# ByteDance-Seed/Bagel

Hardware: NVIDIA H100
Metric: denoised images/sec @1024^2, 50 steps, BAGEL-7B-MoT (higher is better)
Workload: dtype bf16

## Files before the change

### bagel_b200/csrc/attn.cu

```cuda
#include <cuda.h>
#include <cuda_bf16.h>
#include <cuda_runtime.h>
#include <stdint.h>
#include <stdio.h>
#include <stdlib.h>

#include "common.cuh"
#include "host_util.h"
#include "attn_decode.h"

namespace bagel {

constexpr int kAttnThreads = 2 * 128 + 32;
constexpr int kAttnMmaWarps = 8;
constexpr int kBlockM = 128;
constexpr int kBlockN = 128;

struct AttnParams {
  __nv_bfloat16* out;
  long long ld_out;
  const int* cu_q;
  const int* cu_k;
  const int* seqused_k;
  int Hq, Hk;
  int causal;
  float scale_log2;
  int poly;
};

template <int D>
struct AttnCfg {
  static constexpr int kTileBytes = kBlockM * D * 2;
  static constexpr int kStages = (D == 128) ? 4 : 6;
  static constexpr int kSmemBytes = kTileBytes + kStages * kTileBytes + 1024 + 256;
};

__device__ __forceinline__ float ex2(float x) {
  float y;
  asm("ex2.approx.ftz.f32 %0, %1;" : "=f"(y) : "f"(x));
  return y;
}

__device__ __forceinline__ float2 ex2_poly2(float2 x) {
  const float2 magic = make_float2(12582912.0f, 12582912.0f);
  const float2 c1 = make_float2(0.69328292f, 0.69328292f), c2 = make_float2(0.24221068f, 0.24221068f),
               c3 = make_float2(0.05500873f, 0.05500873f);
  x.x = fmaxf(x.x, -126.0f);
  x.y = fmaxf(x.y, -126.0f);
  const float2 t = make_float2(x.x + magic.x, x.y + magic.y);
  const float2 n = make_float2(t.x - magic.x, t.y - magic.y);
  const float2 f = make_float2(x.x - n.x, x.y - n.y);
  float2 q = make_float2(fmaf(f.x, c3.x, c2.x), fmaf(f.y, c3.y, c2.y));
  q = make_float2(fmaf(q.x, f.x, c1.x), fmaf(q.y, f.y, c1.y));
  q = make_float2(fmaf(q.x, f.x, 1.0f), fmaf(q.y, f.y, 1.0f));
  float2 r;
  r.x = __int_as_float(__float_as_int(q.x) + (__float_as_int(t.x) << 23));
  r.y = __int_as_float(__float_as_int(q.y) + (__float_as_int(t.y) << 23));
  return r;
}

template <int D>
__global__ void __launch_bounds__(kAttnThreads, 1)
attn_varlen_kernel(const __grid_constant__ CUtensorMap tmQ, const __grid_constant__ CUtensorMap tmK,
                   const __grid_constant__ CUtensorMap tmV, const AttnParams p) {
  using Cfg = AttnCfg<D>;
  constexpr int kStages = Cfg::kStages;
  constexpr int kTileBytes = Cfg::kTileBytes;
  constexpr int kAtoms = D / 64;
  constexpr int kAtomBytes = kBlockM * 128;

  const int qt = p.causal ? (int)(gridDim.x - 1 - blockIdx.x) : (int)blockIdx.x;
  const int h = blockIdx.y, b = blockIdx.z;
  const int q_beg = p.cu_q[b];
  const int Lq = p.cu_q[b + 1] - q_beg;
  const int q0 = qt * kBlockM;
  if (q0 >= Lq) return;
  const int hk = h / (p.Hq / p.Hk);
  const int k_beg = p.cu_k[b];
  const int Lk = p.seqused_k ? p.seqused_k[b] : (p.cu_k[b + 1] - k_beg);
  const int shift = Lk - Lq;
  int kv_end = Lk;
  if (p.causal) kv_end = max(0, min(Lk, min(Lq, q0 + kBlockM) - 1 + shift + 1));
  const int nblk = (kv_end + kBlockN - 1) / kBlockN;

  extern __shared__ uint8_t smem_raw[];
  uint8_t* smem = reinterpret_cast<uint8_t*>((reinterpret_cast<uintptr_t>(smem_raw) + 1023) & ~uintptr_t(1023));
  uint8_t* smem_q = smem;
  uint8_t* smem_kv = smem + kTileBytes;
  uint64_t* bars = reinterpret_cast<uint64_t*>(smem_kv + kStages * kTileBytes);
  uint64_t* q_full = bars;
  uint64_t* kv_full = bars + 1;
  uint64_t* kv_empty = kv_full + kStages;

  const int wg = threadIdx.x >> 7;
  const int warp = threadIdx.x >> 5;
  const int lane = threadIdx.x & 31;

  if (threadIdx.x == 0) {
    tma_prefetch_desc(&tmQ);
    tma_prefetch_desc(&tmK);
    tma_prefetch_desc(&tmV);
    mbar_init(q_full, 1);
    for (int i = 0; i < kStages; ++i) {
      mbar_init(&kv_full[i], 1);
      mbar_init(&kv_empty[i], kAttnMmaWarps);
    }
    fence_mbar_init();
  }
  __syncthreads();

  if (wg == 2) {
    if (elect_one_lane() && nblk > 0) {
      mbar_expect_tx(q_full, kTileBytes);
      for (int a = 0; a < kAtoms; ++a)
        tma_load_2d(smem_q + a * kAtomBytes, &tmQ, q_full, h * D + a * 64, q_beg + q0, kEvictFirst);
      int stage = 0;
      uint32_t phase = 0;
      for (int j = 0; j < nblk; ++j) {
        for (int kv = 0; kv < 2; ++kv) {
          mbar_wait(&kv_empty[stage], phase ^ 1);
          mbar_expect_tx(&kv_full[stage], kTileBytes);
          const CUtensorMap* tm = kv == 0 ? &tmK : &tmV;
          for (int a = 0; a < kAtoms; ++a)
            tma_load_2d(smem_kv + stage * kTileBytes + a * kAtomBytes, tm, &kv_full[stage], hk * D + a * 64,
                        k_beg + j * kBlockN, kEvictLast);
          if (++stage == kStages) { stage = 0; phase ^= 1; }
        }
      }
    }
  } else {
    const int half = wg;
    const int cq = 2 * (lane & 3);
    const int row0 = half * 64 + (warp & 3) * 16 + (lane >> 2);
    const int qi[2] = {q0 + row0, q0 + row0 + 8};
    float o[D / 2];
#pragma unroll
    for (int i = 0; i < D / 2; ++i) o[i] = 0.f;
    float m[2] = {-INFINITY, -INFINITY}, l[2] = {0.f, 0.f};

    if (nblk > 0) {
      mbar_wait(q_full, 0);
      const uint32_t q_addr = smem_u32(smem_q) + half * 64 * 128;
      const int tile_q_lo = q0 + half * 64;
      int stage = 0;
      uint32_t phase = 0;
      for (int j = 0; j < nblk; ++j) {
        float s[kBlockN / 2];
        mbar_wait(&kv_full[stage], phase);
        {
          const uint32_t k_addr = smem_u32(smem_kv + stage * kTileBytes);
          wgmma_fence();
#pragma unroll
          for (int a = 0; a < kAtoms; ++a)
#pragma unroll
            for (int k = 0; k < 4; ++k)
              wgmma_ss<kBlockN>(s, gmma_desc_kmajor_sw128(q_addr + a * kAtomBytes) + 2 * k,
                                gmma_desc_kmajor_sw128(k_addr + a * kAtomBytes) + 2 * k, (a | k) != 0);
          wgmma_commit();
          wgmma_wait<0>();
          gmma_fence_operand(s);
        }
        __syncwarp();
        if (lane == 0) mbar_arrive(&kv_empty[stage]);
        if (++stage == kStages) { stage = 0; phase ^= 1; }

        const int kv0 = j * kBlockN;
        const bool need_mask = (kv0 + kBlockN > Lk) || (p.causal && (kv0 + kBlockN - 1 > tile_q_lo + shift));
        if (need_mask) {
#pragma unroll
          for (int r = 0; r < 2; ++r) {
            const int lim = p.causal ? min(Lk - 1, qi[r] + shift) : (Lk - 1);
#pragma unroll
            for (int c = 0; c < kBlockN / 8; ++c)
#pragma unroll
              for (int e = 0; e < 2; ++e)
                if (kv0 + 8 * c + cq + e > lim) s[4 * c + 2 * r + e] = -INFINITY;
          }
        }
        float neg_ms[2], alpha[2];
#pragma unroll
        for (int r = 0; r < 2; ++r) {
          float mx = -INFINITY;
#pragma unroll
          for (int c = 0; c < kBlockN / 8; ++c) mx = fmaxf(mx, fmaxf(s[4 * c + 2 * r], s[4 * c + 2 * r + 1]));
          mx = fmaxf(mx, __shfl_xor_sync(0xffffffffu, mx, 1));
          mx = fmaxf(mx, __shfl_xor_sync(0xffffffffu, mx, 2));
          const float m_new = fmaxf(m[r], mx);
          const float m_use = (m_new == -INFINITY) ? 0.f : m_new;
          alpha[r] = ex2((m[r] - m_use) * p.scale_log2);
          m[r] = m_new;
          neg_ms[r] = -m_use * p.scale_log2;
        }
        const bool poly = p.poly && !need_mask;
        float rs[2] = {0.f, 0.f};
        uint32_t pa[kBlockN / 16][4];
#pragma unroll
        for (int c = 0; c < kBlockN / 8; ++c) {
#pragma unroll
          for (int r = 0; r < 2; ++r) {
            const float2 x = make_float2(fmaf(s[4 * c + 2 * r], p.scale_log2, neg_ms[r]),
                                         fmaf(s[4 * c + 2 * r + 1], p.scale_log2, neg_ms[r]));
            const float2 e = (poly && (c & 3) == 3) ? ex2_poly2(x) : make_float2(ex2(x.x), ex2(x.y));
            rs[r] += e.x + e.y;
            pa[c >> 1][(c & 1) * 2 + r] = pack_bf16x2(e.x, e.y);
          }
        }
#pragma unroll
        for (int r = 0; r < 2; ++r) {
          l[r] = l[r] * alpha[r] + rs[r];
#pragma unroll
          for (int c = 0; c < D / 8; ++c) {
            o[4 * c + 2 * r] *= alpha[r];
            o[4 * c + 2 * r + 1] *= alpha[r];
          }
        }

        mbar_wait(&kv_full[stage], phase);
        {
          const uint32_t v_addr = smem_u32(smem_kv + stage * kTileBytes);
          wgmma_fence();
#pragma unroll
          for (int kk = 0; kk < kBlockN / 16; ++kk)
            wgmma_rs<D, 1>(o, pa[kk], gmma_desc_mnmajor_sw128(v_addr + kk * 2048, kAtomBytes), 1u);
          wgmma_commit();
          wgmma_wait<0>();
          gmma_fence_operand(o);
        }
        __syncwarp();
        if (lane == 0) mbar_arrive(&kv_empty[stage]);
        if (++stage == kStages) { stage = 0; phase ^= 1; }
      }
    }

#pragma unroll
    for (int r = 0; r < 2; ++r) {
      float lr = l[r];
      lr += __shfl_xor_sync(0xffffffffu, lr, 1);
      lr += __shfl_xor_sync(0xffffffffu, lr, 2);
      const float inv_l = (lr > 0.f && m[r] != -INFINITY) ? (1.f / lr) : 0.f;
      if (qi[r] >= Lq) continue;
      __nv_bfloat16* orow = p.out + (long long)(q_beg + qi[r]) * p.ld_out + h * D;
#pragma unroll
      for (int c = 0; c < D / 8; ++c)
        *reinterpret_cast<uint32_t*>(orow + 8 * c + cq) = pack_bf16x2(o[4 * c + 2 * r] * inv_l, o[4 * c + 2 * r + 1] * inv_l);
    }
  }
}

template <int D>
static int launch_attn(const CUtensorMap& tmQ, const CUtensorMap& tmK, const CUtensorMap& tmV, const AttnParams& p, int B,
                       int max_seqlen_q, cudaStream_t stream) {
  using Cfg = AttnCfg<D>;
  auto kern = attn_varlen_kernel<D>;
  static bool attr_done = false;
  if (!attr_done) {
    BAGEL_CUDA_CHECK(cudaFuncSetAttribute(kern, cudaFuncAttributeMaxDynamicSharedMemorySize, Cfg::kSmemBytes));
    attr_done = true;
  }
  const int qtiles = (max_seqlen_q + kBlockM - 1) / kBlockM;
  if (p.Hq > 65535 || B > 65535) return set_error(BAGEL_ERR_SHAPE, "bagel_attn_varlen_fwd: too many heads / samples");
  kern<<<dim3(qtiles, p.Hq, B), kAttnThreads, Cfg::kSmemBytes, stream>>>(tmQ, tmK, tmV, p);
  g_launches.fetch_add(1, std::memory_order_relaxed);
  BAGEL_CUDA_CHECK(cudaGetLastError());
  return 0;
}

}

using namespace bagel;

extern "C" int bagel_attn_varlen_fwd(const void* q, const void* k, const void* v, void* out, const int* cu_seqlens_q,
                                     const int* cu_seqlens_k, int total_q, int total_k, int batch, int num_heads_q,
                                     int num_heads_k, int head_dim, int max_seqlen_q, int max_seqlen_k, int causal,
                                     float softmax_scale, long long ld_q, long long ld_k, long long ld_v,
                                     long long ld_out, const int* seqused_k, void* stream) {
  if (head_dim != 64 && head_dim != 128)
    return set_error(BAGEL_ERR_SHAPE, "bagel_attn_varlen_fwd: head_dim must be 64 or 128 (got %d)", head_dim);
  if (num_heads_k <= 0 || num_heads_q % num_heads_k)
    return set_error(BAGEL_ERR_SHAPE, "bagel_attn_varlen_fwd: num_heads_q %% num_heads_k != 0");
  if (batch <= 0 || total_q < 0 || total_k < 0) return set_error(BAGEL_ERR_SHAPE, "bagel_attn_varlen_fwd: bad sizes");
  if ((ld_q % 8) || (ld_k % 8) || (ld_v % 8) || (ld_out % 8) || (((uintptr_t)q | (uintptr_t)k | (uintptr_t)v | (uintptr_t)out) & 15))
    return set_error(BAGEL_ERR_ALIGN, "bagel_attn_varlen_fwd: row strides %% 8 and 16-byte aligned pointers required");
  if (int rc = require_sm90()) return rc;
  if (total_q == 0 || max_seqlen_q <= 0) return 0;
  if (attn_decode_supported(max_seqlen_q, head_dim, num_heads_q, num_heads_k))
    return attn_decode(q, k, v, out, cu_seqlens_q, cu_seqlens_k, seqused_k, batch, num_heads_q, num_heads_k,
                       max_seqlen_k, softmax_scale, ld_q, ld_k, ld_v, ld_out, static_cast<cudaStream_t>(stream));

  CUtensorMap tmQ, tmK, tmV;
  if (int rc = make_tmap_2d_bf16(&tmQ, q, (uint64_t)num_heads_q * head_dim, (uint64_t)total_q, (uint64_t)ld_q, 64, kBlockM)) return rc;
  const uint64_t rows_k = total_k > 0 ? (uint64_t)total_k : 1;
  if (int rc = make_tmap_2d_bf16(&tmK, k, (uint64_t)num_heads_k * head_dim, rows_k, (uint64_t)ld_k, 64, kBlockN)) return rc;
  if (int rc = make_tmap_2d_bf16(&tmV, v, (uint64_t)num_heads_k * head_dim, rows_k, (uint64_t)ld_v, 64, kBlockN)) return rc;

  AttnParams p{};
  p.out = static_cast<__nv_bfloat16*>(out);
  p.ld_out = ld_out;
  p.cu_q = cu_seqlens_q;
  p.cu_k = cu_seqlens_k;
  p.seqused_k = seqused_k;
  p.Hq = num_heads_q;
  p.Hk = num_heads_k;
  p.causal = causal;
  p.scale_log2 = softmax_scale * 1.4426950408889634f;
  static const int poly_env = [] { const char* e = getenv("BAGEL_ATTN_POLY"); return e ? (atoi(e) != 0 ? 1 : 0) : -1; }();
  p.poly = poly_env >= 0 ? poly_env : ((causal || max_seqlen_k < 2048) ? 0 : 1);
  cudaStream_t s = static_cast<cudaStream_t>(stream);
  if (head_dim == 128) return launch_attn<128>(tmQ, tmK, tmV, p, batch, max_seqlen_q, s);
  return launch_attn<64>(tmQ, tmK, tmV, p, batch, max_seqlen_q, s);
}
```

### bagel_b200/csrc/common.cuh

```cuda
#pragma once
#include <cuda.h>
#include <cuda_bf16.h>
#include <cuda_runtime.h>
#include <stdint.h>
#include <stdio.h>

#include "wgmma.cuh"

namespace bagel {

__device__ __forceinline__ uint32_t smem_u32(const void* p) {
  return static_cast<uint32_t>(__cvta_generic_to_shared(p));
}

__device__ __forceinline__ bool elect_one() {
  uint32_t pred = 0;
  asm volatile(
      "{\n\t"
      ".reg .pred P;\n\t"
      "elect.sync _|P, 0xffffffff;\n\t"
      "selp.b32 %0, 1, 0, P;\n\t"
      "}\n"
      : "=r"(pred));
  return pred != 0;
}

__device__ __forceinline__ void mbar_init(uint64_t* bar, uint32_t count) {
  asm volatile("mbarrier.init.shared::cta.b64 [%0], %1;" ::"r"(smem_u32(bar)), "r"(count) : "memory");
}
__device__ __forceinline__ void fence_mbar_init() {
  asm volatile("fence.mbarrier_init.release.cluster;" ::: "memory");
}
__device__ __forceinline__ void mbar_expect_tx(uint64_t* bar, uint32_t bytes) {
  asm volatile("mbarrier.arrive.expect_tx.shared::cta.b64 _, [%0], %1;" ::"r"(smem_u32(bar)), "r"(bytes)
               : "memory");
}
__device__ __forceinline__ void mbar_arrive(uint64_t* bar) {
  asm volatile("mbarrier.arrive.shared::cta.b64 _, [%0];" ::"r"(smem_u32(bar)) : "memory");
}
__device__ __forceinline__ bool mbar_try_wait(uint64_t* bar, uint32_t parity) {
  uint32_t ok;
  asm volatile(
      "{\n\t"
      ".reg .pred P;\n\t"
      "mbarrier.try_wait.parity.shared::cta.b64 P, [%1], %2;\n\t"
      "selp.b32 %0, 1, 0, P;\n\t"
      "}\n"
      : "=r"(ok)
      : "r"(smem_u32(bar)), "r"(parity)
      : "memory");
  return ok != 0;
}
__device__ __forceinline__ void mbar_wait(uint64_t* bar, uint32_t parity) {
  if (mbar_try_wait(bar, parity)) return;
  const long long t0 = clock64();
  while (!mbar_try_wait(bar, parity)) {
    if (clock64() - t0 > 4000000000LL) {
#ifdef BAGEL_MBAR_TRACE
      printf("bagel_b200: mbarrier wait timed out (block %d thread %d bar %u parity %u)\n", blockIdx.x,
             threadIdx.x, smem_u32(bar), parity);
#endif
      __trap();
    }
  }
}

__device__ __forceinline__ uint32_t cluster_ctarank() {
  uint32_t r;
  asm volatile("mov.u32 %0, %%cluster_ctarank;" : "=r"(r));
  return r;
}
__device__ __forceinline__ void cluster_sync_all() {
  asm volatile("barrier.cluster.arrive.release.aligned;" ::: "memory");
  asm volatile("barrier.cluster.wait.acquire.aligned;" ::: "memory");
}
__device__ __forceinline__ uint32_t mapa_shared(uint32_t local_addr, uint32_t rank) {
  uint32_t remote;
  asm volatile("mapa.shared::cluster.u32 %0, %1, %2;" : "=r"(remote) : "r"(local_addr), "r"(rank));
  return remote;
}
__device__ __forceinline__ float ld_dsmem_f32(uint32_t local_addr, uint32_t rank) {
  float v;
  asm volatile("ld.shared::cluster.f32 %0, [%1];" : "=f"(v) : "r"(mapa_shared(local_addr, rank)) : "memory");
  return v;
}
__device__ __forceinline__ void mbar_arrive_cluster(uint64_t* bar, uint32_t rank) {
  asm volatile("mbarrier.arrive.shared::cluster.b64 _, [%0];" ::"r"(mapa_shared(smem_u32(bar), rank)) : "memory");
}

__device__ __forceinline__ bool elect_one_lane() {
  uint32_t pred;
  asm volatile(
      "{\n\t"
      ".reg .pred p;\n\t"
      "elect.sync _|p, 0xffffffff;\n\t"
      "selp.b32 %0, 1, 0, p;\n\t"
      "}\n"
      : "=r"(pred));
  return pred != 0;
}

__device__ __forceinline__ void pdl_launch_dependents() { asm volatile("griddepcontrol.launch_dependents;" ::: "memory"); }
__device__ __forceinline__ void pdl_wait() { asm volatile("griddepcontrol.wait;" ::: "memory"); }

__device__ __forceinline__ void fence_async_smem() {
  asm volatile("fence.proxy.async.shared::cta;" ::: "memory");
}

__device__ __forceinline__ void tma_prefetch_desc(const CUtensorMap* tm) {
  asm volatile("prefetch.tensormap [%0];" ::"l"(reinterpret_cast<uint64_t>(tm)) : "memory");
}
constexpr uint64_t kEvictNormal = 0x1000000000000000ull;
constexpr uint64_t kEvictFirst = 0x12F0000000000000ull;
constexpr uint64_t kEvictLast = 0x14F0000000000000ull;

__device__ __forceinline__ void tma_load_2d(void* smem_dst, const CUtensorMap* tm, uint64_t* bar, int c0, int c1,
                                            uint64_t hint) {
  asm volatile(
      "cp.async.bulk.tensor.2d.shared::cluster.global.mbarrier::complete_tx::bytes.L2::cache_hint"
      " [%0], [%1, {%3, %4}], [%2], %5;"
      ::"r"(smem_u32(smem_dst)),
      "l"(reinterpret_cast<uint64_t>(tm)), "r"(smem_u32(bar)), "r"(c0), "r"(c1), "l"(hint)
      : "memory");
}
__device__ __forceinline__ void tma_load_2d_multicast(void* smem_dst, const CUtensorMap* tm, uint64_t* bar, int c0, int c1,
                                                      uint16_t cta_mask, uint64_t hint) {
  asm volatile(
      "cp.async.bulk.tensor.2d.shared::cluster.global.mbarrier::complete_tx::bytes.multicast::cluster.L2::cache_hint"
      " [%0], [%1, {%3, %4}], [%2], %5, %6;"
      ::"r"(smem_u32(smem_dst)),
      "l"(reinterpret_cast<uint64_t>(tm)), "r"(smem_u32(bar)), "r"(c0), "r"(c1), "h"(cta_mask), "l"(hint)
      : "memory");
}
__device__ __forceinline__ void tma_load_4d(void* smem_dst, const CUtensorMap* tm, uint64_t* bar, int c0, int c1,
                                            int c2, int c3, uint64_t hint) {
  asm volatile(
      "cp.async.bulk.tensor.4d.shared::cluster.global.mbarrier::complete_tx::bytes.L2::cache_hint"
      " [%0], [%1, {%3, %4, %5, %6}], [%2], %7;"
      ::"r"(smem_u32(smem_dst)),
      "l"(reinterpret_cast<uint64_t>(tm)), "r"(smem_u32(bar)), "r"(c0), "r"(c1), "r"(c2), "r"(c3), "l"(hint)
      : "memory");
}
__device__ __forceinline__ void tma_store_2d(const CUtensorMap* tm, const void* smem_src, int c0, int c1) {
  asm volatile("cp.async.bulk.tensor.2d.global.shared::cta.bulk_group [%0, {%2, %3}], [%1];" ::"l"(
                   reinterpret_cast<uint64_t>(tm)),
               "r"(smem_u32(smem_src)), "r"(c0), "r"(c1)
               : "memory");
}
__device__ __forceinline__ void tma_store_commit() { asm volatile("cp.async.bulk.commit_group;" ::: "memory"); }
template <int N>
__device__ __forceinline__ void tma_store_wait_read() {
  asm volatile("cp.async.bulk.wait_group.read %0;" ::"n"(N) : "memory");
}
template <int N>
__device__ __forceinline__ void tma_store_wait() {
  asm volatile("cp.async.bulk.wait_group %0;" ::"n"(N) : "memory");
}

__device__ __forceinline__ uint64_t gmma_desc_kmajor_sw128(uint32_t smem_addr) {
  return (uint64_t)((smem_addr & 0x3FFFF) >> 4) | (1ull << 16) | ((uint64_t)(1024 >> 4) << 32) | (1ull << 62);
}
__device__ __forceinline__ uint64_t gmma_desc_mnmajor_sw128(uint32_t smem_addr, uint32_t lbo_bytes) {
  return (uint64_t)((smem_addr & 0x3FFFF) >> 4) | ((uint64_t)((lbo_bytes >> 4) & 0x3FFF) << 16) |
         ((uint64_t)(1024 >> 4) << 32) | (1ull << 62);
}

template <int N>
__device__ __forceinline__ void gmma_fence_operand(float (&d)[N]) {
#pragma unroll
  for (int i = 0; i < N; ++i) asm volatile("" : "+f"(d[i])::"memory");
}
__device__ __forceinline__ void wgmma_fence() { asm volatile("wgmma.fence.sync.aligned;" ::: "memory"); }
__device__ __forceinline__ void wgmma_commit() { asm volatile("wgmma.commit_group.sync.aligned;" ::: "memory"); }
template <int N>
__device__ __forceinline__ void wgmma_wait() {
  asm volatile("wgmma.wait_group.sync.aligned %0;" ::"n"(N) : "memory");
}

template <int N, int kTnspB = 0>
__device__ __forceinline__ void wgmma_ss(float (&d)[N / 2], uint64_t a_desc, uint64_t b_desc, uint32_t scale_d) {
  if constexpr (N == 16) wgmma_ss_n16<kTnspB>(d, a_desc, b_desc, scale_d);
  else if constexpr (N == 32) wgmma_ss_n32<kTnspB>(d, a_desc, b_desc, scale_d);
  else if constexpr (N == 64) wgmma_ss_n64<kTnspB>(d, a_desc, b_desc, scale_d);
  else if constexpr (N == 128) wgmma_ss_n128<kTnspB>(d, a_desc, b_desc, scale_d);
  else {
    static_assert(N == 256, "wgmma_ss: N in {16, 32, 64, 128, 256}");
    wgmma_ss_n256<kTnspB>(d, a_desc, b_desc, scale_d);
  }
}
template <int N, int kTnspB>
__device__ __forceinline__ void wgmma_rs(float (&d)[N / 2], const uint32_t (&a)[4], uint64_t b_desc, uint32_t scale_d) {
  if constexpr (N == 64) wgmma_rs_n64<kTnspB>(d, a, b_desc, scale_d);
  else {
    static_assert(N == 128, "wgmma_rs: N in {64, 128}");
    wgmma_rs_n128<kTnspB>(d, a, b_desc, scale_d);
  }
}

template <uint32_t kRegs>
__device__ __forceinline__ void setmaxnreg_dec() { asm volatile("setmaxnreg.dec.sync.aligned.u32 %0;" ::"n"(kRegs)); }
template <uint32_t kRegs>
__device__ __forceinline__ void setmaxnreg_inc() { asm volatile("setmaxnreg.inc.sync.aligned.u32 %0;" ::"n"(kRegs)); }

__device__ __forceinline__ float bf16_round(float x) { return __bfloat162float(__float2bfloat16_rn(x)); }
__device__ __forceinline__ uint32_t pack_bf16x2(float lo, float hi) {
  __nv_bfloat162 v = __floats2bfloat162_rn(lo, hi);
  return *reinterpret_cast<uint32_t*>(&v);
}
__device__ __forceinline__ float bf16_lo(uint32_t v) { return __uint_as_float(v << 16); }
__device__ __forceinline__ float bf16_hi(uint32_t v) { return __uint_as_float(v & 0xFFFF0000u); }

}
```

Before: 0.09359.

## Make varlen attention persistent with Q double-use barriers and ping-pong warpgroup scheduling

Converts the attention kernel into a persistent kernel launched with one CTA per SM that loops over flattened (qtile, head, batch) tiles. A q_empty barrier lets the producer reload Q for the next tile while K/V keep streaming. Named barriers alternate the two consumer warpgroups' QK^T wgmma issue so one group's softmax overlaps the other's tensor-core work. This removes per-CTA launch and prologue overhead, but adds barrier handshakes, a required even stage count, and extra paths for inactive half-tiles.

```diff
diff --git a/bagel_b200/csrc/attn.cu b/bagel_b200/csrc/attn.cu
--- a/bagel_b200/csrc/attn.cu
+++ b/bagel_b200/csrc/attn.cu
@@ -1,6 +1,7 @@
 #include <cuda.h>
 #include <cuda_bf16.h>
 #include <cuda_runtime.h>
+#include <limits.h>
 #include <stdint.h>
 #include <stdio.h>
 #include <stdlib.h>
@@ -23,6 +24,9 @@
   const int* cu_k;
   const int* seqused_k;
   int Hq, Hk;
+  int batch;
+  int qtiles;
+  int ntiles;
   int causal;
   float scale_log2;
   int poly;
@@ -59,6 +63,42 @@
   return r;
 }
 
+struct AttnTile {
+  int h, b, hk;
+  int q_beg, Lq, q0;
+  int k_beg, Lk;
+  int shift;
+  int nblk;
+};
+
+__device__ __forceinline__ bool attn_tile(const AttnParams& p, int t, AttnTile& g) {
+  int qt;
+  if (p.causal) {
+    const int hb = p.Hq * p.batch;
+    qt = p.qtiles - 1 - t / hb;
+    t %= hb;
+  } else {
+    qt = t % p.qtiles;
+    t /= p.qtiles;
+  }
+  g.h = t % p.Hq;
+  g.b = t / p.Hq;
+  g.q_beg = p.cu_q[g.b];
+  g.Lq = p.cu_q[g.b + 1] - g.q_beg;
+  g.q0 = qt * kBlockM;
+  if (g.q0 >= g.Lq) return false;
+  g.hk = g.h / (p.Hq / p.Hk);
+  g.k_beg = p.cu_k[g.b];
+  g.Lk = p.seqused_k ? p.seqused_k[g.b] : (p.cu_k[g.b + 1] - g.k_beg);
+  g.shift = g.Lk - g.Lq;
+  int kv_end = g.Lk;
+  if (p.causal) kv_end = max(0, min(g.Lk, min(g.Lq, g.q0 + kBlockM) - 1 + g.shift + 1));
+  g.nblk = (kv_end + kBlockN - 1) / kBlockN;
+  return true;
+}
+
+constexpr uint32_t kBarTurn = 1;
+
 template <int D>
 __global__ void __launch_bounds__(kAttnThreads, 1)
 attn_varlen_kernel(const __grid_constant__ CUtensorMap tmQ, const __grid_constant__ CUtensorMap tmK,
@@ -68,20 +108,7 @@
   constexpr int kTileBytes = Cfg::kTileBytes;
   constexpr int kAtoms = D / 64;
   constexpr int kAtomBytes = kBlockM * 128;
-
-  const int qt = p.causal ? (int)(gridDim.x - 1 - blockIdx.x) : (int)blockIdx.x;
-  const int h = blockIdx.y, b = blockIdx.z;
-  const int q_beg = p.cu_q[b];
-  const int Lq = p.cu_q[b + 1] - q_beg;
-  const int q0 = qt * kBlockM;
-  if (q0 >= Lq) return;
-  const int hk = h / (p.Hq / p.Hk);
-  const int k_beg = p.cu_k[b];
-  const int Lk = p.seqused_k ? p.seqused_k[b] : (p.cu_k[b + 1] - k_beg);
-  const int shift = Lk - Lq;
-  int kv_end = Lk;
-  if (p.causal) kv_end = max(0, min(Lk, min(Lq, q0 + kBlockM) - 1 + shift + 1));
-  const int nblk = (kv_end + kBlockN - 1) / kBlockN;
+  static_assert(kStages % 2 == 0, "K_j and V_j share a ring phase: K at an even stage, V at the next one");
 
   extern __shared__ uint8_t smem_raw[];
   uint8_t* smem = reinterpret_cast<uint8_t*>((reinterpret_cast<uintptr_t>(smem_raw) + 1023) & ~uintptr_t(1023));
@@ -89,7 +116,8 @@
   uint8_t* smem_kv = smem + kTileBytes;
   uint64_t* bars = reinterpret_cast<uint64_t*>(smem_kv + kStages * kTileBytes);
   uint64_t* q_full = bars;
-  uint64_t* kv_full = bars + 1;
+  uint64_t* q_empty = bars + 1;
+  uint64_t* kv_full = bars + 2;
   uint64_t* kv_empty = kv_full + kStages;
 
   const int wg = threadIdx.x >> 7;
@@ -101,6 +129,7 @@
     tma_prefetch_desc(&tmK);
     tma_prefetch_desc(&tmV);
     mbar_init(q_full, 1);
+    mbar_init(q_empty, kAttnMmaWarps);
     for (int i = 0; i < kStages; ++i) {
       mbar_init(&kv_full[i], 1);
       mbar_init(&kv_empty[i], kAttnMmaWarps);
@@ -110,145 +139,178 @@
   __syncthreads();
 
   if (wg == 2) {
-    if (elect_one_lane() && nblk > 0) {
-      mbar_expect_tx(q_full, kTileBytes);
-      for (int a = 0; a < kAtoms; ++a)
-        tma_load_2d(smem_q + a * kAtomBytes, &tmQ, q_full, h * D + a * 64, q_beg + q0, kEvictFirst);
+    if (elect_one_lane()) {
       int stage = 0;
-      uint32_t phase = 0;
-      for (int j = 0; j < nblk; ++j) {
-        for (int kv = 0; kv < 2; ++kv) {
-          mbar_wait(&kv_empty[stage], phase ^ 1);
-          mbar_expect_tx(&kv_full[stage], kTileBytes);
-          const CUtensorMap* tm = kv == 0 ? &tmK : &tmV;
-          for (int a = 0; a < kAtoms; ++a)
-            tma_load_2d(smem_kv + stage * kTileBytes + a * kAtomBytes, tm, &kv_full[stage], hk * D + a * 64,
-                        k_beg + j * kBlockN, kEvictLast);
-          if (++stage == kStages) { stage = 0; phase ^= 1; }
+      uint32_t phase = 0, q_phase = 0;
+      for (int t = blockIdx.x; t < p.ntiles; t += gridDim.x) {
+        AttnTile g;
+        if (!attn_tile(p, t, g) || g.nblk == 0) continue;
+        mbar_wait(q_empty, q_phase ^ 1);
+        q_phase ^= 1;
+        mbar_expect_tx(q_full, kTileBytes);
+        for (int a = 0; a < kAtoms; ++a)
+          tma_load_2d(smem_q + a * kAtomBytes, &tmQ, q_full, g.h * D + a * 64, g.q_beg + g.q0, kEvictFirst);
+        for (int j = 0; j < g.nblk; ++j) {
+          for (int kv = 0; kv < 2; ++kv) {
+            mbar_wait(&kv_empty[stage], phase ^ 1);
+            mbar_expect_tx(&kv_full[stage], kTileBytes);
+            const CUtensorMap* tm = kv == 0 ? &tmK : &tmV;
+            for (int a = 0; a < kAtoms; ++a)
+              tma_load_2d(smem_kv + stage * kTileBytes + a * kAtomBytes, tm, &kv_full[stage], g.hk * D + a * 64,
+                          g.k_beg + j * kBlockN, kEvictLast);
+            if (++stage == kStages) { stage = 0; phase ^= 1; }
+          }
         }
       }
     }
   } else {
-    const int half = wg;
+    const int half = __shfl_sync(0xffffffffu, wg, 0);
     const int cq = 2 * (lane & 3);
     const int row0 = half * 64 + (warp & 3) * 16 + (lane >> 2);
-    const int qi[2] = {q0 + row0, q0 + row0 + 8};
-    float o[D / 2];
-#pragma unroll
-    for (int i = 0; i < D / 2; ++i) o[i] = 0.f;
-    float m[2] = {-INFINITY, -INFINITY}, l[2] = {0.f, 0.f};
-
-    if (nblk > 0) {
-      mbar_wait(q_full, 0);
-      const uint32_t q_addr = smem_u32(smem_q) + half * 64 * 128;
-      const int tile_q_lo = q0 + half * 64;
-      int stage = 0;
-      uint32_t phase = 0;
-      for (int j = 0; j < nblk; ++j) {
-        float s[kBlockN / 2];
-        mbar_wait(&kv_full[stage], phase);
-        {
-          const uint32_t k_addr = smem_u32(smem_kv + stage * kTileBytes);
-          wgmma_fence();
-#pragma unroll
-          for (int a = 0; a < kAtoms; ++a)
-#pragma unroll
-            for (int k = 0; k < 4; ++k)
-              wgmma_ss<kBlockN>(s, gmma_desc_kmajor_sw128(q_addr + a * kAtomBytes) + 2 * k,
-                                gmma_desc_kmajor_sw128(k_addr + a * kAtomBytes) + 2 * k, (a | k) != 0);
-          wgmma_commit();
+    const uint32_t q_addr = smem_u32(smem_q) + half * 64 * 128;
+    int stage = 0;
+    uint32_t phase = 0, q_phase = 0;
+    if (half == 1) named_bar_arrive(kBarTurn, 256);
+
+    for (int t = blockIdx.x; t < p.ntiles; t += gridDim.x) {
+      AttnTile g;
+      if (!attn_tile(p, t, g)) continue;
+      const int qi[2] = {g.q0 + row0, g.q0 + row0 + 8};
+      const int tile_q_lo = g.q0 + half * 64;
+      const bool active = tile_q_lo < g.Lq;
+      float o[D / 2];
+#pragma unroll
+      for (int i = 0; i < D / 2; ++i) o[i] = 0.f;
+      float m[2] = {-INFINITY, -INFINITY}, l[2] = {0.f, 0.f};
+
+      if (g.nblk > 0 && !active) {
+        for (int j = 0; j < g.nblk; ++j) {
+          named_bar_sync(kBarTurn + 1, 256);
+          named_bar_arrive(kBarTurn, 256);
+          if (lane == 0) {
+            mbar_arrive(&kv_empty[stage]);
+            mbar_arrive(&kv_empty[stage + 1]);
+            if (j == g.nblk - 1) mbar_arrive(q_empty);
+          }
+          if ((stage += 2) == kStages) { stage = 0; phase ^= 1; }
+        }
+        q_phase ^= 1;
+      } else if (g.nblk > 0) {
+        mbar_wait(q_full, q_phase);
+        for (int j = 0; j < g.nblk; ++j) {
+          float s[kBlockN / 2];
+          mbar_wait(&kv_full[stage], phase);
+          if (half == 0) named_bar_sync(kBarTurn, 256); else named_bar_sync(kBarTurn + 1, 256);
+          {
+            const uint32_t k_addr = smem_u32(smem_kv + stage * kTileBytes);
+            wgmma_fence();
+#pragma unroll
+            for (int a = 0; a < kAtoms; ++a)
+#pragma unroll
+              for (int k = 0; k < 4; ++k)
+                wgmma_ss<kBlockN>(s, gmma_desc_kmajor_sw128(q_addr + a * kAtomBytes) + 2 * k,
+                                  gmma_desc_kmajor_sw128(k_addr + a * kAtomBytes) + 2 * k, (a | k) != 0);
+            wgmma_commit();
+          }
+          if (half == 0) named_bar_arrive(kBarTurn + 1, 256); else named_bar_arrive(kBarTurn, 256);
           wgmma_wait<0>();
           gmma_fence_operand(s);
+          __syncwarp();
+          if (lane == 0) {
+            mbar_arrive(&kv_empty[stage]);
+            if (j == g.nblk - 1) mbar_arrive(q_empty);
+          }
+
+          const int kv0 = j * kBlockN;
+          const bool need_mask = (kv0 + kBlockN > g.Lk) || (p.causal && (kv0 + kBlockN - 1 > tile_q_lo + g.shift));
+          if (need_mask) {
+#pragma unroll
+            for (int r = 0; r < 2; ++r) {
+              const int lim = p.causal ? min(g.Lk - 1, qi[r] + g.shift) : (g.Lk - 1);
+#pragma unroll
+              for (int c = 0; c < kBlockN / 8; ++c)
+#pragma unroll
+                for (int e = 0; e < 2; ++e)
+                  if (kv0 + 8 * c + cq + e > lim) s[4 * c + 2 * r + e] = -INFINITY;
+            }
+          }
+          float neg_ms[2], alpha[2];
+#pragma unroll
+          for (int r = 0; r < 2; ++r) {
+            float mx = -INFINITY;
+#pragma unroll
+            for (int c = 0; c < kBlockN / 8; ++c) mx = fmaxf(mx, fmaxf(s[4 * c + 2 * r], s[4 * c + 2 * r + 1]));
+            mx = fmaxf(mx, __shfl_xor_sync(0xffffffffu, mx, 1));
+            mx = fmaxf(mx, __shfl_xor_sync(0xffffffffu, mx, 2));
+            const float m_new = fmaxf(m[r], mx);
+            const float m_use = (m_new == -INFINITY) ? 0.f : m_new;
+            alpha[r] = ex2((m[r] - m_use) * p.scale_log2);
+            m[r] = m_new;
+            neg_ms[r] = -m_use * p.scale_log2;
+          }
+          const bool poly = p.poly && !need_mask;
+          float rs[2] = {0.f, 0.f};
+          uint32_t pa[kBlockN / 16][4];
+#pragma unroll
+          for (int c = 0; c < kBlockN / 8; ++c) {
+#pragma unroll
+            for (int r = 0; r < 2; ++r) {
+              const float2 x = make_float2(fmaf(s[4 * c + 2 * r], p.scale_log2, neg_ms[r]),
+                                           fmaf(s[4 * c + 2 * r + 1], p.scale_log2, neg_ms[r]));
+              const float2 e = (poly && (c & 3) == 3) ? ex2_poly2(x) : make_float2(ex2(x.x), ex2(x.y));
+              rs[r] += e.x + e.y;
+              pa[c >> 1][(c & 1) * 2 + r] = pack_bf16x2(e.x, e.y);
+            }
+          }
+#pragma unroll
+          for (int r = 0; r < 2; ++r) {
+            l[r] = l[r] * alpha[r] + rs[r];
+#pragma unroll
+            for (int c = 0; c < D / 8; ++c) {
+              o[4 * c + 2 * r] *= alpha[r];
+              o[4 * c + 2 * r + 1] *= alpha[r];
+            }
+          }
+
+          mbar_wait(&kv_full[stage + 1], phase);
+          {
+            const uint32_t v_addr = smem_u32(smem_kv + (stage + 1) * kTileBytes);
+            wgmma_fence();
+#pragma unroll
+            for (int kk = 0; kk < kBlockN / 16; ++kk)
+              wgmma_rs<D, 1>(o, pa[kk], gmma_desc_mnmajor_sw128(v_addr + kk * 2048, kAtomBytes), 1u);
+            wgmma_commit();
+            wgmma_wait<0>();
+            gmma_fence_operand(o);
+          }
+          __syncwarp();
+          if (lane == 0) mbar_arrive(&kv_empty[stage + 1]);
+          if ((stage += 2) == kStages) { stage = 0; phase ^= 1; }
         }
-        __syncwarp();
-        if (lane == 0) mbar_arrive(&kv_empty[stage]);
-        if (++stage == kStages) { stage = 0; phase ^= 1; }
-
-        const int kv0 = j * kBlockN;
-        const bool need_mask = (kv0 + kBlockN > Lk) || (p.causal && (kv0 + kBlockN - 1 > tile_q_lo + shift));
-        if (need_mask) {
-#pragma unroll
-          for (int r = 0; r < 2; ++r) {
-            const int lim = p.causal ? min(Lk - 1, qi[r] + shift) : (Lk - 1);
-#pragma unroll
-            for (int c = 0; c < kBlockN / 8; ++c)
-#pragma unroll
-              for (int e = 0; e < 2; ++e)
-                if (kv0 + 8 * c + cq + e > lim) s[4 * c + 2 * r + e] = -INFINITY;
-          }
-        }
-        float neg_ms[2], alpha[2];
-#pragma unroll
-        for (int r = 0; r < 2; ++r) {
-          float mx = -INFINITY;
-#pragma unroll
-          for (int c = 0; c < kBlockN / 8; ++c) mx = fmaxf(mx, fmaxf(s[4 * c + 2 * r], s[4 * c + 2 * r + 1]));
-          mx = fmaxf(mx, __shfl_xor_sync(0xffffffffu, mx, 1));
-          mx = fmaxf(mx, __shfl_xor_sync(0xffffffffu, mx, 2));
-          const float m_new = fmaxf(m[r], mx);
-          const float m_use = (m_new == -INFINITY) ? 0.f : m_new;
-          alpha[r] = ex2((m[r] - m_use) * p.scale_log2);
-          m[r] = m_new;
-          neg_ms[r] = -m_use * p.scale_log2;
-        }
-        const bool poly = p.poly && !need_mask;
-        float rs[2] = {0.f, 0.f};
-        uint32_t pa[kBlockN / 16][4];
-#pragma unroll
-        for (int c = 0; c < kBlockN / 8; ++c) {
-#pragma unroll
-          for (int r = 0; r < 2; ++r) {
-            const float2 x = make_float2(fmaf(s[4 * c + 2 * r], p.scale_log2, neg_ms[r]),
-                                         fmaf(s[4 * c + 2 * r + 1], p.scale_log2, neg_ms[r]));
-            const float2 e = (poly && (c & 3) == 3) ? ex2_poly2(x) : make_float2(ex2(x.x), ex2(x.y));
-            rs[r] += e.x + e.y;
-            pa[c >> 1][(c & 1) * 2 + r] = pack_bf16x2(e.x, e.y);
-          }
-        }
-#pragma unroll
-        for (int r = 0; r < 2; ++r) {
-          l[r] = l[r] * alpha[r] + rs[r];
-#pragma unroll
-          for (int c = 0; c < D / 8; ++c) {
-            o[4 * c + 2 * r] *= alpha[r];
-            o[4 * c + 2 * r + 1] *= alpha[r];
-          }
-        }
-
-        mbar_wait(&kv_full[stage], phase);
-        {
-          const uint32_t v_addr = smem_u32(smem_kv + stage * kTileBytes);
-          wgmma_fence();
-#pragma unroll
-          for (int kk = 0; kk < kBlockN / 16; ++kk)
-            wgmma_rs<D, 1>(o, pa[kk], gmma_desc_mnmajor_sw128(v_addr + kk * 2048, kAtomBytes), 1u);
-          wgmma_commit();
-          wgmma_wait<0>();
-          gmma_fence_operand(o);
-        }
-        __syncwarp();
-        if (lane == 0) mbar_arrive(&kv_empty[stage]);
-        if (++stage == kStages) { stage = 0; phase ^= 1; }
+        q_phase ^= 1;
+      }
+
+      attn_tile(p, t, g);
+#pragma unroll
+      for (int r = 0; r < 2; ++r) {
+        float lr = l[r];
+        lr += __shfl_xor_sync(0xffffffffu, lr, 1);
+        lr += __shfl_xor_sync(0xffffffffu, lr, 2);
+        const float inv_l = (lr > 0.f && m[r] != -INFINITY) ? (1.f / lr) : 0.f;
+        if (qi[r] >= g.Lq) continue;
+        __nv_bfloat16* orow = p.out + (long long)(g.q_beg + qi[r]) * p.ld_out + g.h * D;
+#pragma unroll
+        for (int c = 0; c < D / 8; ++c)
+          *reinterpret_cast<uint32_t*>(orow + 8 * c + cq) =
+              pack_bf16x2(o[4 * c + 2 * r] * inv_l, o[4 * c + 2 * r + 1] * inv_l);
       }
     }
-
-#pragma unroll
-    for (int r = 0; r < 2; ++r) {
-      float lr = l[r];
-      lr += __shfl_xor_sync(0xffffffffu, lr, 1);
-      lr += __shfl_xor_sync(0xffffffffu, lr, 2);
-      const float inv_l = (lr > 0.f && m[r] != -INFINITY) ? (1.f / lr) : 0.f;
-      if (qi[r] >= Lq) continue;
-      __nv_bfloat16* orow = p.out + (long long)(q_beg + qi[r]) * p.ld_out + h * D;
-#pragma unroll
-      for (int c = 0; c < D / 8; ++c)
-        *reinterpret_cast<uint32_t*>(orow + 8 * c + cq) = pack_bf16x2(o[4 * c + 2 * r] * inv_l, o[4 * c + 2 * r + 1] * inv_l);
-    }
+    if (half == 0) named_bar_sync(kBarTurn, 256);
   }
 }
 
 template <int D>
-static int launch_attn(const CUtensorMap& tmQ, const CUtensorMap& tmK, const CUtensorMap& tmV, const AttnParams& p, int B,
+static int launch_attn(const CUtensorMap& tmQ, const CUtensorMap& tmK, const CUtensorMap& tmV, AttnParams p,
                        int max_seqlen_q, cudaStream_t stream) {
   using Cfg = AttnCfg<D>;
   auto kern = attn_varlen_kernel<D>;
@@ -257,9 +319,14 @@
     BAGEL_CUDA_CHECK(cudaFuncSetAttribute(kern, cudaFuncAttributeMaxDynamicSharedMemorySize, Cfg::kSmemBytes));
     attr_done = true;
   }
-  const int qtiles = (max_seqlen_q + kBlockM - 1) / kBlockM;
-  if (p.Hq > 65535 || B > 65535) return set_error(BAGEL_ERR_SHAPE, "bagel_attn_varlen_fwd: too many heads / samples");
-  kern<<<dim3(qtiles, p.Hq, B), kAttnThreads, Cfg::kSmemBytes, stream>>>(tmQ, tmK, tmV, p);
+  p.qtiles = (max_seqlen_q + kBlockM - 1) / kBlockM;
+  const long long ntiles = (long long)p.qtiles * p.Hq * p.batch;
+  if (ntiles > INT_MAX) return set_error(BAGEL_ERR_SHAPE, "bagel_attn_varlen_fwd: too many query tiles");
+  p.ntiles = (int)ntiles;
+  static const int max_ctas_env = [] { const char* e = getenv("BAGEL_ATTN_MAX_CTAS"); return e ? atoi(e) : 0; }();
+  int grid = min(sm_count(), p.ntiles);
+  if (max_ctas_env > 0) grid = min(grid, max_ctas_env);
+  kern<<<grid, kAttnThreads, Cfg::kSmemBytes, stream>>>(tmQ, tmK, tmV, p);
   g_launches.fetch_add(1, std::memory_order_relaxed);
   BAGEL_CUDA_CHECK(cudaGetLastError());
   return 0;
@@ -301,11 +368,12 @@
   p.seqused_k = seqused_k;
   p.Hq = num_heads_q;
   p.Hk = num_heads_k;
+  p.batch = batch;
   p.causal = causal;
   p.scale_log2 = softmax_scale * 1.4426950408889634f;
   static const int poly_env = [] { const char* e = getenv("BAGEL_ATTN_POLY"); return e ? (atoi(e) != 0 ? 1 : 0) : -1; }();
   p.poly = poly_env >= 0 ? poly_env : ((causal || max_seqlen_k < 2048) ? 0 : 1);
   cudaStream_t s = static_cast<cudaStream_t>(stream);
-  if (head_dim == 128) return launch_attn<128>(tmQ, tmK, tmV, p, batch, max_seqlen_q, s);
-  return launch_attn<64>(tmQ, tmK, tmV, p, batch, max_seqlen_q, s);
-}
+  if (head_dim == 128) return launch_attn<128>(tmQ, tmK, tmV, p, max_seqlen_q, s);
+  return launch_attn<64>(tmQ, tmK, tmV, p, max_seqlen_q, s);
+}
diff --git a/bagel_b200/csrc/common.cuh b/bagel_b200/csrc/common.cuh
--- a/bagel_b200/csrc/common.cuh
+++ b/bagel_b200/csrc/common.cuh
@@ -100,6 +100,13 @@
   return pred != 0;
 }
 
+__device__ __forceinline__ void named_bar_sync(uint32_t id, uint32_t nthreads) {
+  asm volatile("bar.sync %0, %1;" ::"r"(id), "r"(nthreads) : "memory");
+}
+__device__ __forceinline__ void named_bar_arrive(uint32_t id, uint32_t nthreads) {
+  asm volatile("bar.arrive %0, %1;" ::"r"(id), "r"(nthreads) : "memory");
+}
+
 __device__ __forceinline__ void pdl_launch_dependents() { asm volatile("griddepcontrol.launch_dependents;" ::: "memory"); }
 __device__ __forceinline__ void pdl_wait() { asm volatile("griddepcontrol.wait;" ::: "memory"); }
 
```

After: 0.09405 (median of 6 runs). About the same (+0.5%).

## Add ping-pong scheduling between MMA warpgroups in varlen attention

Applied to the files above, without the earlier changes.

Splits the attention loop into QK+softmax and PV helpers and reorders it so that iteration j runs PV for block j-1 before QK for block j. Named barriers alternate the two consumer warpgroups, so one group's tensor-core GEMMs can run while the other does its softmax. This aims to hide the exp/max work behind the other group's wgmma. The cost is extra barrier synchronisation and tighter coupling between the warpgroups, which could stall if the two groups' per-block work is uneven.

```diff
diff --git a/bagel_b200/csrc/attn.cu b/bagel_b200/csrc/attn.cu
--- a/bagel_b200/csrc/attn.cu
+++ b/bagel_b200/csrc/attn.cu
@@ -15,6 +15,7 @@
 constexpr int kAttnMmaWarps = 8;
 constexpr int kBlockM = 128;
 constexpr int kBlockN = 128;
+constexpr int kAtomBytes = kBlockM * 128;
 
 struct AttnParams {
   __nv_bfloat16* out;
@@ -59,6 +60,68 @@
   return r;
 }
 
+__device__ __forceinline__ void softmax_block(float (&s)[kBlockN / 2], uint32_t (&pa)[kBlockN / 16][4], float (&m)[2],
+                                              float (&alpha)[2], float (&rs)[2], const AttnParams& p, int kv0, int Lk,
+                                              int shift, int tile_q_lo, const int (&qi)[2], int cq) {
+  const bool need_mask = (kv0 + kBlockN > Lk) || (p.causal && (kv0 + kBlockN - 1 > tile_q_lo + shift));
+  if (need_mask) {
+#pragma unroll
+    for (int r = 0; r < 2; ++r) {
+      const int lim = p.causal ? min(Lk - 1, qi[r] + shift) : (Lk - 1);
+#pragma unroll
+      for (int c = 0; c < kBlockN / 8; ++c)
+#pragma unroll
+        for (int e = 0; e < 2; ++e)
+          if (kv0 + 8 * c + cq + e > lim) s[4 * c + 2 * r + e] = -INFINITY;
+    }
+  }
+  float neg_ms[2];
+#pragma unroll
+  for (int r = 0; r < 2; ++r) {
+    float mx = -INFINITY;
+#pragma unroll
+    for (int c = 0; c < kBlockN / 8; ++c) mx = fmaxf(mx, fmaxf(s[4 * c + 2 * r], s[4 * c + 2 * r + 1]));
+    mx = fmaxf(mx, __shfl_xor_sync(0xffffffffu, mx, 1));
+    mx = fmaxf(mx, __shfl_xor_sync(0xffffffffu, mx, 2));
+    const float m_new = fmaxf(m[r], mx);
+    const float m_use = (m_new == -INFINITY) ? 0.f : m_new;
+    alpha[r] = ex2((m[r] - m_use) * p.scale_log2);
+    m[r] = m_new;
+    neg_ms[r] = -m_use * p.scale_log2;
+  }
+  const bool poly = p.poly && !need_mask;
+  rs[0] = rs[1] = 0.f;
+#pragma unroll
+  for (int c = 0; c < kBlockN / 8; ++c) {
+#pragma unroll
+    for (int r = 0; r < 2; ++r) {
+      const float2 x = make_float2(fmaf(s[4 * c + 2 * r], p.scale_log2, neg_ms[r]),
+                                   fmaf(s[4 * c + 2 * r + 1], p.scale_log2, neg_ms[r]));
+      const float2 e = (poly && (c & 3) == 3) ? ex2_poly2(x) : make_float2(ex2(x.x), ex2(x.y));
+      rs[r] += e.x + e.y;
+      pa[c >> 1][(c & 1) * 2 + r] = pack_bf16x2(e.x, e.y);
+    }
+  }
+}
+
+template <int D>
+__device__ __forceinline__ void issue_qk(float (&s)[kBlockN / 2], uint32_t q_addr, uint32_t k_addr) {
+  asm volatile("" : "+r"(q_addr));
+#pragma unroll
+  for (int a = 0; a < D / 64; ++a)
+#pragma unroll
+    for (int k = 0; k < 4; ++k)
+      wgmma_ss<kBlockN>(s, gmma_desc_kmajor_sw128(q_addr + a * kAtomBytes) + 2 * k,
+                        gmma_desc_kmajor_sw128(k_addr + a * kAtomBytes) + 2 * k, (a | k) != 0);
+}
+
+template <int D>
+__device__ __forceinline__ void issue_pv(float (&o)[D / 2], const uint32_t (&pa)[kBlockN / 16][4], uint32_t v_addr) {
+#pragma unroll
+  for (int kk = 0; kk < kBlockN / 16; ++kk)
+    wgmma_rs<D, 1>(o, pa[kk], gmma_desc_mnmajor_sw128(v_addr + kk * 2048, kAtomBytes), 1u);
+}
+
 template <int D>
 __global__ void __launch_bounds__(kAttnThreads, 1)
 attn_varlen_kernel(const __grid_constant__ CUtensorMap tmQ, const __grid_constant__ CUtensorMap tmK,
@@ -67,7 +130,6 @@
   constexpr int kStages = Cfg::kStages;
   constexpr int kTileBytes = Cfg::kTileBytes;
   constexpr int kAtoms = D / 64;
-  constexpr int kAtomBytes = kBlockM * 128;
 
   const int qt = p.causal ? (int)(gridDim.x - 1 - blockIdx.x) : (int)blockIdx.x;
   const int h = blockIdx.y, b = blockIdx.z;
@@ -144,67 +206,29 @@
       const int tile_q_lo = q0 + half * 64;
       int stage = 0;
       uint32_t phase = 0;
-      for (int j = 0; j < nblk; ++j) {
-        float s[kBlockN / 2];
+      auto acquire = [&]() {
         mbar_wait(&kv_full[stage], phase);
-        {
-          const uint32_t k_addr = smem_u32(smem_kv + stage * kTileBytes);
-          wgmma_fence();
-#pragma unroll
-          for (int a = 0; a < kAtoms; ++a)
-#pragma unroll
-            for (int k = 0; k < 4; ++k)
-              wgmma_ss<kBlockN>(s, gmma_desc_kmajor_sw128(q_addr + a * kAtomBytes) + 2 * k,
-                                gmma_desc_kmajor_sw128(k_addr + a * kAtomBytes) + 2 * k, (a | k) != 0);
-          wgmma_commit();
-          wgmma_wait<0>();
-          gmma_fence_operand(s);
-        }
+        return smem_u32(smem_kv + stage * kTileBytes);
+      };
+      auto release = [&]() {
         __syncwarp();
         if (lane == 0) mbar_arrive(&kv_empty[stage]);
         if (++stage == kStages) { stage = 0; phase ^= 1; }
-
-        const int kv0 = j * kBlockN;
-        const bool need_mask = (kv0 + kBlockN > Lk) || (p.causal && (kv0 + kBlockN - 1 > tile_q_lo + shift));
-        if (need_mask) {
-#pragma unroll
-          for (int r = 0; r < 2; ++r) {
-            const int lim = p.causal ? min(Lk - 1, qi[r] + shift) : (Lk - 1);
-#pragma unroll
-            for (int c = 0; c < kBlockN / 8; ++c)
-#pragma unroll
-              for (int e = 0; e < 2; ++e)
-                if (kv0 + 8 * c + cq + e > lim) s[4 * c + 2 * r + e] = -INFINITY;
-          }
-        }
-        float neg_ms[2], alpha[2];
-#pragma unroll
-        for (int r = 0; r < 2; ++r) {
-          float mx = -INFINITY;
-#pragma unroll
-          for (int c = 0; c < kBlockN / 8; ++c) mx = fmaxf(mx, fmaxf(s[4 * c + 2 * r], s[4 * c + 2 * r + 1]));
-          mx = fmaxf(mx, __shfl_xor_sync(0xffffffffu, mx, 1));
-          mx = fmaxf(mx, __shfl_xor_sync(0xffffffffu, mx, 2));
-          const float m_new = fmaxf(m[r], mx);
-          const float m_use = (m_new == -INFINITY) ? 0.f : m_new;
-          alpha[r] = ex2((m[r] - m_use) * p.scale_log2);
-          m[r] = m_new;
-          neg_ms[r] = -m_use * p.scale_log2;
-        }
-        const bool poly = p.poly && !need_mask;
-        float rs[2] = {0.f, 0.f};
-        uint32_t pa[kBlockN / 16][4];
-#pragma unroll
-        for (int c = 0; c < kBlockN / 8; ++c) {
-#pragma unroll
-          for (int r = 0; r < 2; ++r) {
-            const float2 x = make_float2(fmaf(s[4 * c + 2 * r], p.scale_log2, neg_ms[r]),
-                                         fmaf(s[4 * c + 2 * r + 1], p.scale_log2, neg_ms[r]));
-            const float2 e = (poly && (c & 3) == 3) ? ex2_poly2(x) : make_float2(ex2(x.x), ex2(x.y));
-            rs[r] += e.x + e.y;
-            pa[c >> 1][(c & 1) * 2 + r] = pack_bf16x2(e.x, e.y);
-          }
-        }
+      };
+      if (half == 0) named_bar_arrive(1, 256);
+      float s[kBlockN / 2];
+      uint32_t pa[kBlockN / 16][4];
+      auto qk_softmax = [&](int j) {
+        const uint32_t k_addr = acquire();
+        wgmma_fence();
+        issue_qk<D>(s, q_addr, k_addr);
+        wgmma_commit();
+        named_bar_arrive(2 - half, 256);
+        wgmma_wait<0>();
+        gmma_fence_operand(s);
+        release();
+        float alpha[2], rs[2];
+        softmax_block(s, pa, m, alpha, rs, p, j * kBlockN, Lk, shift, tile_q_lo, qi, cq);
 #pragma unroll
         for (int r = 0; r < 2; ++r) {
           l[r] = l[r] * alpha[r] + rs[r];
@@ -214,22 +238,27 @@
             o[4 * c + 2 * r + 1] *= alpha[r];
           }
         }
-
-        mbar_wait(&kv_full[stage], phase);
-        {
-          const uint32_t v_addr = smem_u32(smem_kv + stage * kTileBytes);
-          wgmma_fence();
-#pragma unroll
-          for (int kk = 0; kk < kBlockN / 16; ++kk)
-            wgmma_rs<D, 1>(o, pa[kk], gmma_desc_mnmajor_sw128(v_addr + kk * 2048, kAtomBytes), 1u);
-          wgmma_commit();
-          wgmma_wait<0>();
-          gmma_fence_operand(o);
-        }
-        __syncwarp();
-        if (lane == 0) mbar_arrive(&kv_empty[stage]);
-        if (++stage == kStages) { stage = 0; phase ^= 1; }
+      };
+      auto pv = [&]() {
+        const uint32_t v_addr = acquire();
+        wgmma_fence();
+        issue_pv<D>(o, pa, v_addr);
+        wgmma_commit();
+        wgmma_wait<0>();
+        gmma_fence_operand(o);
+        release();
+      };
+
+      named_bar_sync(1 + half, 256);
+      qk_softmax(0);
+      for (int j = 1; j < nblk; ++j) {
+        named_bar_sync(1 + half, 256);
+        pv();
+        qk_softmax(j);
       }
+      named_bar_sync(1 + half, 256);
+      pv();
+      named_bar_arrive(2 - half, 256);
     }
 
 #pragma unroll
diff --git a/bagel_b200/csrc/common.cuh b/bagel_b200/csrc/common.cuh
--- a/bagel_b200/csrc/common.cuh
+++ b/bagel_b200/csrc/common.cuh
@@ -103,6 +103,13 @@
 __device__ __forceinline__ void pdl_launch_dependents() { asm volatile("griddepcontrol.launch_dependents;" ::: "memory"); }
 __device__ __forceinline__ void pdl_wait() { asm volatile("griddepcontrol.wait;" ::: "memory"); }
 
+__device__ __forceinline__ void named_bar_sync(uint32_t id, uint32_t nthreads) {
+  asm volatile("bar.sync %0, %1;" ::"r"(id), "r"(nthreads) : "memory");
+}
+__device__ __forceinline__ void named_bar_arrive(uint32_t id, uint32_t nthreads) {
+  asm volatile("bar.arrive %0, %1;" ::"r"(id), "r"(nthreads) : "memory");
+}
+
 __device__ __forceinline__ void fence_async_smem() {
   asm volatile("fence.proxy.async.shared::cta;" ::: "memory");
 }
```

Result: no change. 0.09374 before, 0.09453 after (median of 6 runs) (+0.8%).
